# kiranchhatre/amuse

Hardware: AMD Instinct MI355X
Metric: SMPL-X frames/sec (10 s clip, 1000-step DDPM) (higher is better)
Workload: dtype bf16; 1 GPU; 256 x 10 s clips in total (256 on rank 0), DDPM-1000 sampling loop + VAE decode (300 frames) + 6D->axis-angle; random-init weights of the diff_latent_v2 / prior_emotional_fing architecture; clips_total=256, clips_rank0=256, clips_per_tile=2, sampler=ddpm-1000, mfma_operands=bf16, state_and_accumulate=fp32

## Files before the change

### amuse_amd/csrc/amuse_sample8.hpp

```cpp
#pragma once
#include "amuse_dev.hpp"
#include "amuse_kernels.hpp"

namespace amuse {
namespace {

constexpr int kR8 = kRing8;
using Ring = WRing<kR8>;
constexpr int kA8Bytes = 8 * kTiles * 64 * 16;
constexpr int kStat8Off = kA8Bytes;

__device__ __forceinline__ f32x4* a8_slot(char* lds, int row, int col, int lane) {
    return reinterpret_cast<f32x4*>(lds) + (row * kTiles + col) * 64 + lane;
}
__device__ __forceinline__ constexpr int part_row(int w, int t) {
    const int red = 4 + (t >> 1);
    const int k = w - (w > red ? 1 : 0);
    return k + (k >= t ? 1 : 0);
}
__device__ __forceinline__ f32x4* u_slot(char* lds, int t, int lane) { return a8_slot(lds, t == 6 ? 5 : 6, t, lane); }

struct Prof8 {
    unsigned long long* out;
    int idx;
    bool on;
};
template <bool PROF>
__device__ __forceinline__ void stamp8(Prof8& pf) {
    if constexpr (PROF) {
        if (pf.on) pf.out[pf.idx++] = __builtin_readcyclecounter();
    }
}

struct Lane8 {
    int lane, g, r, cl, tok;
    long clip;
    bool valid, is_lat;
};
__device__ __forceinline__ Lane8 lane_info(const SampleKernelArgs& a, int lane) {
    asm volatile("" : "+v"(lane));
    Lane8 L;
    L.lane = lane;
    L.g = lane >> 4;
    L.r = lane & 15;
    const int S = a.S, R = S * a.G;
    L.cl = L.r / S;
    L.tok = L.r - L.cl * S;
    L.clip = (long)blockIdx.x * a.G + L.cl;
    L.valid = (L.r < R) && (L.clip < (long)a.B);
    L.is_lat = L.valid && L.tok == 0;
    return L;
}

__device__ __forceinline__ void store_tap_tile(float* tap, int slot, int t, const f32x4& v, int g, int r) {
    st4(tap + ((size_t)slot * 16 + r) * kD + 16 * t + 4 * g, v);
}

__device__ __forceinline__ bool key_valid8(const Lane8& L0, int j, int S, int R) {
    return L0.valid ? (j < R && (j / S) == L0.cl) : (j == L0.r);
}

__device__ __forceinline__ float2 row_stats32(const f32x4 (&y)[2]) {
    float s = ((y[0][0] + y[0][1]) + (y[0][2] + y[0][3])) + ((y[1][0] + y[1][1]) + (y[1][2] + y[1][3]));
    s = allreduce_g_sum(s);
    const float mw = s * (1.0f / 32.0f);
    float m2 = 0.f;
#pragma unroll
    for (int i = 0; i < 2; ++i)
#pragma unroll
        for (int m = 0; m < 4; ++m) {
            const float d = y[i][m] - mw;
            m2 += d * d;
        }
    m2 = allreduce_g_sum(m2);
    return float2{mw, m2};
}
template <bool FAST>
__device__ __forceinline__ float2 row_stats_merge(const float2* stats, int r) {
    const float2 s0 = stats[r], s1 = stats[16 + r], s2 = stats[32 + r], s3 = stats[48 + r];
    const float mean = ((s0.x + s1.x) + (s2.x + s3.x)) * 0.25f;
    const float d0 = s0.x - mean, d1 = s1.x - mean, d2 = s2.x - mean, d3 = s3.x - mean;
    const float M2 = ((s0.y + s1.y) + (s2.y + s3.y)) + 32.0f * ((d0 * d0 + d1 * d1) + (d2 * d2 + d3 * d3));
    const float var = M2 * (1.0f / kD) + 1e-5f;
    return float2{mean, FAST ? __builtin_amdgcn_rsqf(var) : 1.0f / sqrtf(var)};
}

template <class Args>
__device__ __forceinline__ f32x4 static_row4(const Args& a, const Lane8& L, int f) {
    f32x4 sv = splat4(0.f);
    if (L.valid) {
        if (L.tok == 0) sv = ld4(a.pe0 + f);
        else if (L.tok >= 2) sv = ld4(a.cond_tok + ((size_t)L.clip * (a.S - 2) + (L.tok - 2)) * kD + f);
    }
    return sv;
}
template <class Args>
__device__ __forceinline__ f32x4 init_latent4(const Args& a, const Lane8& L, int t, int f) {
    f32x4 l0 = splat4(0.f);
    if (L.is_lat)
        l0 = a.x_init ? ld4(a.x_init + (size_t)L.clip * kD + f)
                      : counter_normal4(a.seed, a.clip0 + (uint64_t)L.clip, 0u, (uint32_t)(4 * t + L.g), 0u);
    return l0;
}
template <class Args>
__device__ __forceinline__ f32x4 assemble_tile(const Args& a, const Lane8& L, int lane, int g, const f32x4* tokrows, const float* ttl,
                                               const f32x4* latl, int step, int t) {
    const f32x4 sv = tokrows[t * 64 + lane];
    f32x4 tt = ld4(ttl + (step & 1) * kD + 16 * t + 4 * g);
    if (a.time_tok_clip) tt = ld4(a.time_tok_clip + (size_t)(L.valid ? L.clip : 0) * kD + 16 * t + 4 * g);
    return !L.valid ? splat4(0.f) : (L.tok == 0 ? latl[t * 64 + lane] + sv : (L.tok == 1 ? tt : sv));
}

}
}
```

### amuse_amd/csrc/k_sampler8.hip

```cpp
#include "amuse_sample8.hpp"

#ifdef AMUSE_OP_F16
#define OPV f16x8
#define OP_PACK pack_f16
#define OP_MFMA mfma_f16
#define OP_PREC PREC_F16
#define OP_GELU gelu_poly4h
#define OP_KERNEL k_sample8h
#define OP_LAUNCH launch_sample8h
#else
#define OPV bf16x8
#define OP_PACK pack_bf16
#define OP_MFMA mfma_bf16
#define OP_PREC PREC_BF16
#define OP_GELU gelu_poly4
#define OP_KERNEL k_sample8
#define OP_LAUNCH launch_sample8
#endif

namespace amuse {

namespace {

constexpr int kSkip8Off = kStat8Off + 8 * 16 * 8;
// ... 44 lines not shown
            ga[i] = ld4(gamma + 16 * (T0 + i) + 4 * g);
            be[i] = ld4(beta + 16 * (T0 + i) + 4 * g);
        }
    }
    __syncthreads();
    f32x4 y[2];
    {
        f32x4 p[NP][2];
#pragma unroll
        for (int i = 0; i < 2; ++i)
#pragma unroll
            for (int w = 0; w < NP; ++w) {
                if (w != 4 + W) p[w][i] = *a8_slot(lds, part_row(w, T0 + i), T0 + i, lane);
            }
#pragma unroll
        for (int i = 0; i < 2; ++i) {
            f32x4 sum;
            if constexpr (NP == 8) {
                p[4 + W][i] = part[T0 + i];
                sum = ((p[0][i] + p[1][i]) + (p[2][i] + p[3][i])) + ((p[4][i] + p[5][i]) + (p[6][i] + p[7][i]));
            } else {
                sum = ((p[0][i] + p[1][i]) + p[2][i]) + p[3][i];
            }
            f32x4 br = sum + bi[i];
            if constexpr (DRP) br = sdrop_apply4(br, dbits >> (4 * i), dscale);
            y[i] = LN ? xo[i] + br : br;
        }
    }
    if constexpr (LN) {
    const float2 st = row_stats32(y);
    if (g == 0) stats[W * 16 + r] = st;
    __syncthreads();
    const float2 ms = row_stats_merge<FAST>(stats, r);
    const float mean = ms.x, rstd = ms.y;
#pragma unroll
    for (int i = 0; i < 2; ++i)
#pragma unroll
        for (int m = 0; m < 4; ++m) y[i][m] = (y[i][m] - mean) * rstd * ga[i][m] + be[i][m];
    }
    xo[0] = y[0];
    xo[1] = y[1];
    xb[W] = OP_PACK(y[0], y[1]);
    *xb_slot(lds, W, lane) = __builtin_bit_cast(uint4, xb[W]);
    __syncthreads();
#pragma unroll
    for (int c = 0; c < 4; ++c)
        if (c != W) xb[c] = __builtin_bit_cast(OPV, *xb_slot(lds, c, lane));
    asm volatile("; combine_red case %0" ::"n"(W));
}
template <int NP, bool FAST, bool LN = true, bool DRP = false>
__device__ __forceinline__ void combine_reduce(f32x4 (&part)[kTiles], f32x4 (&xo)[2], OPV (&xb)[4],
                                               const float* bias, const float* gamma, const float* beta, char* lds,
                                               int h, int lane, uint32_t dbits = 0, float dscale = 1.f) {
    if (h == 0) combine_red<0, NP, FAST, LN, DRP>(part, xo, xb, bias, gamma, beta, lds, lane, dbits, dscale);
    else if (h == 1) combine_red<1, NP, FAST, LN, DRP>(part, xo, xb, bias, gamma, beta, lds, lane, dbits, dscale);
    else if (h == 2) combine_red<2, NP, FAST, LN, DRP>(part, xo, xb, bias, gamma, beta, lds, lane, dbits, dscale);
    else combine_red<3, NP, FAST, LN, DRP>(part, xo, xb, bias, gamma, beta, lds, lane, dbits, dscale);
}
struct NoHook {
    __device__ void operator()() const {}
};
template <int N0, int N1, int N2, int N3, int IPH0, bool LN = true, class Hook = NoHook>
__device__ __forceinline__ void combine_publish(const f32x4 (&part)[kTiles], OPV (&xb)[4], char* lds, int h,
                                                int lane, Ring& rg, Hook hook = {}) {
#pragma unroll
    for (int t = 0; t < kTiles; ++t)
        *a8_slot(lds, h + (h >= t ? 1 : 0), t, lane) = part[t];
    ring_issue<N0, kR8, IPH0 % kR8>(rg);
    __syncthreads();
    ring_issue<N1, kR8, (IPH0 + N0) % kR8>(rg);
    hook();
    if constexpr (LN) __syncthreads();
    ring_issue<N2, kR8, (IPH0 + N0 + N1) % kR8>(rg);
    __syncthreads();
#pragma unroll
    for (int c = 0; c < 4; ++c) xb[c] = __builtin_bit_cast(OPV, *xb_slot(lds, c, lane));
    ring_issue<N3, kR8, (IPH0 + N0 + N1 + N2) % kR8>(rg);
}

template <int N0, int N1, int N2>
__device__ __forceinline__ void combine_publish_c2(const f32x4 (&part)[kTiles], OPV (&xb)[4], char* lds, int h,
                                                   int lane, Ring& rg, bool skip_u, const uint4* skip_ops) {
    static_assert(N0 >= 8 && N0 + N1 + N2 == 32, "the leading 8 units go out before the first barrier");
#pragma unroll
    for (int t = 0; t < kTiles; ++t)
        *a8_slot(lds, h + (h >= t ? 1 : 0), t, lane) = part[t];
    ring_issue<N0, kR8, 24>(rg);
    __syncthreads();
    ring_issue<N1, kR8, (24 + N0) % kR8>(rg);
    __syncthreads();
    if (skip_u) {
        OPV sk[4];
#pragma unroll
        for (int p = 0; p < 4; ++p) sk[p] = __builtin_bit_cast(OPV, skip_ops[p * 64 + lane]);
        f32x4 u[2] = {splat4(0.f), splat4(0.f)};
        gemm_xb<2, false, 24>(u, sk, rg);
        *u_slot(lds, 2 * h, lane) = u[0];
        *u_slot(lds, 2 * h + 1, lane) = u[1];
    }
    ring_issue<N2, kR8, (24 + N0 + N1) % kR8>(rg);
    __syncthreads();
#pragma unroll
    for (int c = 0; c < 4; ++c) xb[c] = __builtin_bit_cast(OPV, *xb_slot(lds, c, lane));
}

template <bool DROP = false>
__device__ __forceinline__ void attention_head8(const f32x4 (&q)[2], const f32x4 (&k)[2], const f32x4 (&v)[2],
                                                const bool (&kvalid)[4], f32x4 (&o)[2], uint32_t dbits = 0,
                                                float dscale = 1.f) {
    f32x4 st = OP_MFMA(OP_PACK(k[0], k[1]), OP_PACK(q[0], q[1]), splat4(0.f));
    float mx = -INFINITY;
#pragma unroll
    for (int m = 0; m < 4; ++m) mx = kvalid[m] ? fmaxf(mx, st[m]) : mx;
    mx = allreduce_g_max(mx);
    f32x4 p;
    float sum = 0.f;
#pragma unroll
    for (int m = 0; m < 4; ++m) {
        const float e = __builtin_amdgcn_exp2f(1.44269504088896340736f * (st[m] - mx));
        p[m] = kvalid[m] ? e : 0.f;
        sum += p[m];
    }
    sum = allreduce_g_sum(sum);
    const float inv = __builtin_amdgcn_rcpf(sum);
#pragma unroll
    for (int m = 0; m < 4; ++m) p[m] *= inv;
    if constexpr (DROP) p = sdrop_apply4(p, dbits, dscale);
#pragma unroll
    for (int td = 0; td < 2; ++td)
        o[td] = OP_MFMA(OP_PACK(v[td], splat4(0.f)), OP_PACK(p, splat4(0.f)), splat4(0.f));
}

template <bool DROP>
__device__ __forceinline__ void gelu_pair(f32x4 (&hq)[2], uint32_t dbits, float dscale) {
    hq[0] = OP_GELU(hq[0]);
    hq[1] = OP_GELU(hq[1]);
    if constexpr (DROP) {
        hq[0] = sdrop_apply4(hq[0], dbits, dscale);
        hq[1] = sdrop_apply4(hq[1], dbits >> 4, dscale);
    }
}

template <int Q0, int NLATE, bool DROP = false>
__device__ __forceinline__ void ffn_half(f32x4 (&part)[kTiles], const OPV (&xb)[4], Ring& rg, const float* pv,
                                         int h, int g, uint32_t dbits = 0, float dscale = 1.f) {
    constexpr int P = OP_PREC;
    const float* b1 = pv + PV_L1_B + 16 * (kTiles * h + 2 * Q0) + 4 * g;
    f32x4 ha[2] = {ld4(b1), ld4(b1 + 16)}, hb[2] = {ld4(b1 + 32), ld4(b1 + 48)};
    gemm_xb<2, false, 0>(ha, xb, rg);
    ring_issue<NLATE, kR8, 32 - NLATE>(rg);
    __builtin_amdgcn_sched_barrier(0);
    gemm_xb<2, false, 8>(hb, xb, rg);
    gelu_pair<DROP>(ha, dbits, dscale);
#pragma unroll
    for (int i = 0; i < 8; ++i) {
        __builtin_amdgcn_sched_group_barrier(0x008, 1, 0);
        __builtin_amdgcn_sched_group_barrier(0x002, kFfnValuPerMfma, 0);
    }
    __builtin_amdgcn_sched_barrier(0);
    gemm_ring<P, kTiles, 2, false, kR8, 16, false>(part, ha, rg);
    gelu_pair<DROP>(hb, dbits >> 8, dscale);
#pragma unroll
    for (int i = 0; i < 8; ++i) {
        __builtin_amdgcn_sched_group_barrier(0x008, 1, 0);
        __builtin_amdgcn_sched_group_barrier(0x002, kFfnValuPerMfma, 0);
    }
    __builtin_amdgcn_sched_barrier(0);
    gemm_ring<P, kTiles, 2, false, kR8, 24, false>(part, hb, rg);
}

struct SDrop8 {
    uint64_t seed;
    uint32_t step, epoch2, thr;
    float scale;
};
template <bool DROP, class Args>
__device__ __forceinline__ SDrop8 sdrop8_of(const Args& a) {
    SDrop8 d{};
    if constexpr (DROP) {
        d.seed = a.drop_seed; d.epoch2 = 2u + *a.drop_epoch; d.thr = a.drop_thr; d.scale = a.drop_scale;
    }
    return d;
}
__device__ __forceinline__ uint32_t sdrop8_attn_bits(const SampleKernelArgs& a, const SDrop8& d, int blk, int h, int lane) {
    const Lane8 L = lane_info(a, lane);
    const int S = a.S, base = (h * S + L.tok) * S + 4 * L.g - L.cl * S, e4 = base >> 2;
    const uint32_t cu = (uint32_t)(a.clip0 + (uint64_t)L.clip), ls = 4u * blk;
    const uint32_t b = sdrop_bits4(d.seed, cu, d.step, ls, (uint32_t)e4 & 0xffffu, d.epoch2, d.thr) |
                       (sdrop_bits4(d.seed, cu, d.step, ls, (uint32_t)(e4 + 1) & 0xffffu, d.epoch2, d.thr) << 4);
    return b >> (base - 4 * e4);
}
template <int Q0>
__device__ __forceinline__ uint32_t sdrop8_ffn_bits(const SampleKernelArgs& a, const SDrop8& d, int blk, int h, int lane) {
    const Lane8 L = lane_info(a, lane);
    const uint32_t cu = (uint32_t)(a.clip0 + (uint64_t)L.clip), e4 = (uint32_t)(L.tok * 128 + 4 * (kTiles * h + 2 * Q0) + L.g);
    uint32_t b = 0;
#pragma unroll
    for (int k = 0; k < 4; ++k) b |= sdrop_bits4(d.seed, cu, d.step, 4u * blk + 2u, e4 + 4 * k, d.epoch2, d.thr) << (4 * k);
    return b;
}
__device__ __forceinline__ uint32_t sdrop8_row_bits(const SampleKernelArgs& a, const SDrop8& d, uint32_t ls, int h, int lane) {
    const Lane8 L = lane_info(a, lane);
    const uint32_t cu = (uint32_t)(a.clip0 + (uint64_t)L.clip), e4 = (uint32_t)(L.tok * 32 + 8 * h + L.g);
    return sdrop_bits4(d.seed, cu, d.step, ls, e4, d.epoch2, d.thr) | (sdrop_bits4(d.seed, cu, d.step, ls, e4 + 4, d.epoch2, d.thr) << 4);
}

template <bool ROLEA, bool PROF, bool DROP, class Early = NoHook>
__device__ __forceinline__ void encoder_block8(OPV (&xb)[4], f32x4 (&xo)[2], Ring& rg, const float* pv,
                                               const bool (&kvalid)[4], char* lds, int h, int lane, bool next_has_skip,
                                               const uint4* skip_next, Prof8& pf, const SampleKernelArgs& a,
                                               const SDrop8& dr, int blk, Early early = {}) {
    constexpr int P = OP_PREC;
    const int g = lane >> 4, r = lane & 15;
    f32x4 part[kTiles];
    if constexpr (ROLEA) {
        uint32_t abits = 0, fbits = 0;
        if constexpr (DROP) abits = sdrop8_attn_bits(a, dr, blk, h, lane);
        f32x4 b_qk[4];
        float b_v[2];
#pragma unroll
        for (int o = 0; o < 2; ++o) {
            b_qk[o] = ld4(pv + PV_IN_B + 16 * (2 * h + o) + 4 * g);
            b_qk[2 + o] = ld4(pv + PV_IN_B + kD + 16 * (2 * h + o) + 4 * g);
            b_v[o] = pv[PV_IN_B + 2 * kD + 16 * (2 * h + o) + r];
        }
        f32x4 qk[4], v[2];
#pragma unroll
        for (int o = 0; o < 4; ++o) qk[o] = splat4(0.f);
        v[0] = v[1] = splat4(0.f);
        gemm_xb<4, false, 0>(qk, xb, rg);
        gemm_xb<2, true, 16>(v, xb, rg);
        const float scaling = 0.17677669529663687f;
        f32x4 q[2] = {(qk[0] + b_qk[0]) * scaling, (qk[1] + b_qk[1]) * scaling};
        f32x4 k[2] = {qk[2] + b_qk[2], qk[3] + b_qk[3]};
        v[0] += splat4(b_v[0]);
        v[1] += splat4(b_v[1]);
        f32x4 o[2];
        attention_head8<DROP>(q, k, v, kvalid, o, abits, dr.scale);
#pragma unroll
        for (int t = 0; t < kTiles; ++t) part[t] = splat4(0.f);
        gemm_ring<P, kTiles, 2, false, kR8, 24, false>(part, o, rg);
        stamp8<PROF>(pf);
        if constexpr (DROP) {
            auto hook = [&]() { fbits = sdrop8_ffn_bits<0>(a, dr, blk, h, lane); };
            combine_publish<0, kC1N1, kC1N2, 32 - kC1N1 - kC1N2 - kALate, 0, true, decltype(hook)>(part, xb, lds, h, lane, rg, hook);
        } else {
            combine_publish<0, kC1N1, kC1N2, 32 - kC1N1 - kC1N2 - kALate, 0>(part, xb, lds, h, lane, rg);
        }
        stamp8<PROF>(pf);
#pragma unroll
        for (int t = 0; t < kTiles; ++t) part[t] = splat4(0.f);
        ffn_half<0, kALate, DROP>(part, xb, rg, pv, h, g, fbits, dr.scale);
        stamp8<PROF>(pf);
        combine_publish_c2<kC2N0, kC2N1, 32 - kC2N0 - kC2N1>(part, xb, lds, h, lane, rg, next_has_skip, skip_next);
    } else {
        ring_issue<kBEarly, kR8, 0>(rg);
        early();
        uint32_t bbits = 0;
        if constexpr (DROP)
            bbits = sdrop8_row_bits(a, dr, 4u * blk + 1u, h, lane) | (sdrop8_row_bits(a, dr, 4u * blk + 3u, h, lane) << 8) |
                    (sdrop8_ffn_bits<2>(a, dr, blk, h, lane) << 16);
        stamp8<PROF>(pf);
#pragma unroll
        for (int t = 0; t < kTiles; ++t) part[t] = splat4(0.f);
        combine_reduce<4, true, true, DROP>(part, xo, xb, pv + PV_OUT_B, pv + PV_LN1_W, pv + PV_LN1_B, lds, h, lane, bbits, dr.scale);
        stamp8<PROF>(pf);
        ffn_half<2, 32 - kBEarly, DROP>(part, xb, rg, pv, h, g, bbits >> 16, dr.scale);
        stamp8<PROF>(pf);
        if (next_has_skip) ring_issue<8, kR8, 0>(rg);
        combine_reduce<8, true, true, DROP>(part, xo, xb, pv + PV_L2_B, pv + PV_LN2_W, pv + PV_LN2_B, lds, h, lane, bbits >> 8, dr.scale);
    }
    stamp8<PROF>(pf);
}

template <bool ROLEA, bool PROF, bool DROP, class Args>
__device__ __forceinline__ void role_loop8(const Args& a, char* smem, int w8, const Lane8& L0) {
    uint4* skipbf = reinterpret_cast<uint4*>(smem + kSkip8Off);
    const float* pvl = reinterpret_cast<const float*>(smem + kPv8Off);
    const f32x4* tokrows = reinterpret_cast<const f32x4*>(smem + kTokRows8Off);
    f32x4* latl = reinterpret_cast<f32x4*>(smem + kLat8Off);
    float* ttl = reinterpret_cast<float*>(smem + kTT8Off);
    float2* stats = reinterpret_cast<float2*>(smem + kStat8Off);
    const float* pv_skip = pvl + kLayers * kEncPv;
    const float* pv_final = pv_skip + 4 * kD;
    const int lane = L0.lane, g = L0.g, r = L0.r, h = w8 & 3;
    const int S = a.S, R = S * a.G;
    bool kvalid[4];
#pragma unroll
    for (int m = 0; m < 4; ++m) kvalid[m] = key_valid8(L0, 4 * g + m, S, R);
    const bool tap = !ROLEA && a.tap_out != nullptr && blockIdx.x == 0;
    const uint32_t wbase_units = ROLEA ? (uint32_t)w8 * (a.wave_units_a + kR8)
                                       : 4u * (a.wave_units_a + kR8) + (uint32_t)(w8 - 4) * a.wave_units_b;
    const uint4* wbase = a.wstream + (size_t)wbase_units * 64 + lane;
    Ring rg;
    if constexpr (ROLEA) {
#pragma unroll
        for (int i = 0; i < kR8; ++i) rg.s[(24 + i) % kR8] = ldw(wbase + i * 64);
        rg.next = wbase + kR8 * 64;
    } else {
        ring_fill(rg, wbase);
    }
    Prof8 pf{a.prof_out ? a.prof_out + (size_t)w8 * 96 : nullptr, 0, false};
    SDrop8 dr = sdrop8_of<DROP>(a);
#pragma unroll 1
    for (int step = 0; step < a.T; ++step) {
        dr.step = (uint32_t)step;
        OPV xb[4];
        f32x4 xo[2] = {splat4(0.f), splat4(0.f)};
        f32x4 zn[2] = {splat4(0.f), splat4(0.f)};
        {
            const Lane8 L = lane_info(a, lane);
            auto assemble = [&](int t) { return assemble_tile(a, L, lane, g, tokrows, ttl, latl, step, t); };
#pragma unroll
            for (int c = 0; c < 4; ++c) xb[c] = OP_PACK(assemble(2 * c), assemble(2 * c + 1));
            if constexpr (!ROLEA) {
                xo[0] = assemble(2 * h);
                xo[1] = assemble(2 * h + 1);
            }
        }
        if (tap && step == 0) {
            store_tap_tile(a.tap_out, 0, 2 * h, xo[0], g, r);
            store_tap_tile(a.tap_out, 0, 2 * h + 1, xo[1], g, r);
        }
        if (!ROLEA && w8 == 4 && lane < 32 && step + 1 < a.T)
            st4(ttl + ((step + 1) & 1) * kD + 4 * lane, ld4(a.time_tok + (size_t)(step + 1) * kD + 4 * lane));
        if constexpr (PROF) {
            pf.on = a.prof_out != nullptr && blockIdx.x == 0 && lane == 0 && step == a.prof_step;
            pf.idx = 0;
        }
        stamp8<PROF>(pf);
        rg.next = ROLEA ? wbase + kR8 * 64 : wbase;
#pragma unroll 1
        for (int blk = 0; blk < kLayers; ++blk) {
            if (blk >= 5) {
                if constexpr (ROLEA) {
                    ring_issue<8, kR8, 24>(rg);
                } else {
                    const float* bs = pv_skip + (blk - 5) * kD + 32 * h + 4 * g;
                    f32x4 acc[2] = {ld4(bs) + *u_slot(smem, 2 * h, lane), ld4(bs + 16) + *u_slot(smem, 2 * h + 1, lane)};
                    gemm_xb<2, false, 0>(acc, xb, rg);
                    xo[0] = acc[0];
                    xo[1] = acc[1];
                    *reinterpret_cast<uint4*>(a8_slot(smem, 7, h, lane)) = __builtin_bit_cast(uint4, OP_PACK(acc[0], acc[1]));
                }
                __syncthreads();
#pragma unroll
                for (int c = 0; c < 4; ++c) xb[c] = __builtin_bit_cast(OPV, *reinterpret_cast<const uint4*>(a8_slot(smem, 7, c, lane)));
            }
            stamp8<PROF>(pf);
            auto early = [&]() {
                if constexpr (!ROLEA && !DROP) {
                    if (blk == kLayers - 1 && !a.no_update && !a.step_noise) {
                        const Lane8 L = lane_info(a, lane);
                        if (a.coef[(size_t)step * 8 + 5] != 0.f && L.is_lat) {
#pragma unroll
                            for (int i = 0; i < 2; ++i)
                                zn[i] = counter_normal4(a.seed, a.clip0 + (uint64_t)L.clip, (uint32_t)step, (uint32_t)(4 * (2 * h + i) + L.g), 1u);
                        }
                    }
                }
            };
            encoder_block8<ROLEA, PROF, DROP, decltype(early)>(xb, xo, rg, pvl + blk * kEncPv, kvalid, smem, h, lane, blk >= 4 && blk < kLayers - 1,
                                                               skipbf + (7 - blk) * 4 * 64, pf, a, dr, blk, early);
            if (!ROLEA && blk < 4 && w8 == 4) {
#pragma unroll
                for (int p = 0; p < 4; ++p) skipbf[(blk * 4 + p) * 64 + lane] = __builtin_bit_cast(uint4, xb[p]);
            }
            if (tap && step == 0) {
                store_tap_tile(a.tap_out, 1 + blk, 2 * h, xo[0], g, r);
                store_tap_tile(a.tap_out, 1 + blk, 2 * h + 1, xo[1], g, r);
            }
        }
        if constexpr (!ROLEA) {
            const float* cf = a.coef + (size_t)step * 8;
            const float sb = cf[0], sa = cf[1], c0 = cf[2], cx = cf[3], ce = cf[4], sg = cf[5], clipv = cf[6];
            const float2 st = row_stats32(xo);
            if (g == 0) stats[h * 16 + r] = st;
            __syncthreads();
            const Lane8 L = lane_info(a, lane);
            f32x4 ga[2], be[2], l[2];
#pragma unroll
            for (int i = 0; i < 2; ++i) {
                ga[i] = ld4(pv_final + 16 * (2 * h + i) + 4 * L.g);
                be[i] = ld4(pv_final + kD + 16 * (2 * h + i) + 4 * L.g);
                l[i] = latl[(2 * h + i) * 64 + L.lane];
            }
            const float2 ms = row_stats_merge<true>(stats, L.r);
            const float inv_sa = 1.0f / sa;
            f32x4 e[2];
#pragma unroll
            for (int i = 0; i < 2; ++i)
#pragma unroll
                for (int m = 0; m < 4; ++m) e[i][m] = (xo[i][m] - ms.x) * ms.y * ga[i][m] + be[i][m];
#pragma unroll
            for (int i = 0; i < 2; ++i) {
                const int t = 2 * h + i, f = 16 * t + 4 * L.g;
                if (tap && step == 0) store_tap_tile(a.tap_out, 10, t, e[i], L.g, L.r);
                if (a.eps_out && L.is_lat && step == a.T - 1) st4(a.eps_out + (size_t)L.clip * kD + f, e[i]);
            }
            if (!a.no_update) {
                f32x4 z[2] = {zn[0], zn[1]};
                if (sg != 0.f && L.is_lat && (DROP || a.step_noise)) {
#pragma unroll
                    for (int i = 0; i < 2; ++i) {
                        const int t = 2 * h + i, f = 16 * t + 4 * L.g;
                        z[i] = a.step_noise ? ld4(a.step_noise + ((size_t)step * a.B + L.clip) * kD + f)
                                            : counter_normal4(a.seed, a.clip0 + (uint64_t)L.clip, (uint32_t)step, (uint32_t)(4 * t + L.g), 1u);
                    }
                }
#pragma unroll
                for (int i = 0; i < 2; ++i)
#pragma unroll
                    for (int m = 0; m < 4; ++m) l[i][m] = sched_update<true>(l[i][m], e[i][m], z[i][m], sb, sa, c0, cx, ce, sg, clipv, inv_sa);
#pragma unroll
                for (int i = 0; i < 2; ++i) {
                    const int t = 2 * h + i, f = 16 * t + 4 * L.g;
                    latl[t * 64 + L.lane] = l[i];
                    if (a.traj_out && L.is_lat) st4(a.traj_out + ((size_t)step * a.B + L.clip) * kD + f, l[i]);
                }
            }
        } else {
            __syncthreads();
        }
        stamp8<PROF>(pf);
        __syncthreads();
    }
}

template <bool PROF, bool DROP, class Args>
__global__ __launch_bounds__(512) void OP_KERNEL(Args a) {
    extern __shared__ __attribute__((aligned(16))) char smem[];
    float* pvl = reinterpret_cast<float*>(smem + kPv8Off);
    f32x4* tokrows = reinterpret_cast<f32x4*>(smem + kTokRows8Off);
    f32x4* latl = reinterpret_cast<f32x4*>(smem + kLat8Off);
    float* ttl = reinterpret_cast<float*>(smem + kTT8Off);
    for (int i = threadIdx.x; i < kLayers * kEncPv / 4; i += 512) {
        const int blk = (4 * i) / kEncPv, off = 4 * i - blk * kEncPv;
        st4(pvl + 4 * i, ld4(a.pvec + blk * PV_BLOCK + off));
    }
    for (int i = threadIdx.x; i < (4 * kD + 2 * kD) / 4; i += 512) st4(pvl + kLayers * kEncPv + 4 * i, ld4(a.pvec + PV_SKIP_B + 4 * i));
    const int w8 = __builtin_amdgcn_readfirstlane(threadIdx.x >> 6);
    const Lane8 L = lane_info(a, threadIdx.x & 63);
    if (w8 == 0) {
#pragma unroll
        for (int t = 0; t < kTiles; ++t) {
            const int f = 16 * t + 4 * L.g;
            const f32x4 sv = static_row4(a, L, f), l0 = init_latent4(a, L, t, f);
            tokrows[t * 64 + L.lane] = sv;
            latl[t * 64 + L.lane] = l0;
        }
    }
    if (w8 == 4 && L.lane < 32 && !a.time_tok_clip) st4(ttl + 4 * L.lane, ld4(a.time_tok + 4 * L.lane));
    __syncthreads();
    if (w8 < 4) role_loop8<true, PROF, DROP>(a, smem, w8, L);
    else role_loop8<false, PROF, DROP>(a, smem, w8, L);
    if (L.is_lat && w8 == 0 && a.latents_out) {
#pragma unroll
        for (int t = 0; t < kTiles; ++t) st4(a.latents_out + (size_t)L.clip * kD + 16 * t + 4 * L.g, latl[t * 64 + L.lane]);
    }
}

}

hipError_t OP_LAUNCH(const SampleArgs& a_in, hipStream_t stream) {
    SampleArgs a = a_in;
    if (a.drop_thr > 0 && !(a.drop_epoch = train_epoch_ptr())) return hipErrorOutOfMemory;
    const int tiles = (a.B + a.G - 1) / a.G;
    static DeviceOnce once;
    int dev_;
    if (!once.done(&dev_)) {
        for (const void* k : {reinterpret_cast<const void*>(&OP_KERNEL<false, false, SampleKernelArgs>), reinterpret_cast<const void*>(&OP_KERNEL<true, false, SampleKernelArgs>),
                              reinterpret_cast<const void*>(&OP_KERNEL<false, true, SampleArgs>), reinterpret_cast<const void*>(&OP_KERNEL<true, true, SampleArgs>)}) {
            hipError_t e = hipFuncSetAttribute(k, hipFuncAttributeMaxDynamicSharedMemorySize, kSample8LdsBytes);
            if (e != hipSuccess) return e;
        }
        once.set(dev_);
    }
    const SampleKernelArgs ka = a;
    if (a.drop_thr > 0) {
        if (a.prof_out) hipLaunchKernelGGL((OP_KERNEL<true, true, SampleArgs>), dim3(tiles), dim3(512), kSample8LdsBytes, stream, a);
        else hipLaunchKernelGGL((OP_KERNEL<false, true, SampleArgs>), dim3(tiles), dim3(512), kSample8LdsBytes, stream, a);
    } else if (a.prof_out) hipLaunchKernelGGL((OP_KERNEL<true, false, SampleKernelArgs>), dim3(tiles), dim3(512), kSample8LdsBytes, stream, ka);
    else hipLaunchKernelGGL((OP_KERNEL<false, false, SampleKernelArgs>), dim3(tiles), dim3(512), kSample8LdsBytes, stream, ka);
    return hipGetLastError();
}

}
```

### amuse_amd/csrc/k_sampler8x.hip

```cpp
#include "amuse_sample8.hpp"

namespace amuse {

namespace {

constexpr int kPvSlotFloats = 7 * 256;
static_assert(kPvSlotFloats >= kEncPv && kPvSlotFloats <= PV_BLOCK, "a slot is filled by whole pieces read from the block's own region");
constexpr int kPv8Off = kStat8Off + 8 * 16 * 8;
constexpr int kPvTail8Off = kPv8Off + 2 * kPvSlotFloats * 4;
constexpr int kSkip8Off = kPvTail8Off + (4 * kD + 2 * kD) * 4;
constexpr int kTokRows8Off = kSkip8Off + 4 * 8 * 64 * 16;
constexpr int kLat8Off = kTokRows8Off + kTiles * 64 * 16;
constexpr int kTT8Off = kLat8Off + kTiles * 64 * 16;
static_assert(kTT8Off + 2 * kD * 4 == kSample8xLdsBytes, "LDS layout");

constexpr int kXC1N1 = 12, kXC1N2 = 12, kXC2N1 = 8;
constexpr int kXBEarly = 32;
constexpr int kXBPrio = 3;

__device__ __forceinline__ uint4* xs_hi_slot(char* lds, int c, int lane) { return reinterpret_cast<uint4*>(a8_slot(lds, c, c, lane)); }
__device__ __forceinline__ uint4* xs_lo_slot(char* lds, int c, int lane) { return reinterpret_cast<uint4*>(a8_slot(lds, 4 + c, 4 + c, lane)); }
__device__ __forceinline__ void publish_xs(char* lds, int c, int lane, const F16Pair& p) {
    *xs_hi_slot(lds, c, lane) = __builtin_bit_cast(uint4, p.hi);
    *xs_lo_slot(lds, c, lane) = __builtin_bit_cast(uint4, p.lo);
// ... 15 lines not shown
            const int s0 = (PH + 2 * (c * NO + o)) % kR8, s1 = (PH + 2 * (c * NO + o) + 1) % kR8;
            wh[o] = __builtin_bit_cast(f16x8, rg.s[s0]);
            wl[o] = __builtin_bit_cast(f16x8, rg.s[s1]);
            if constexpr (REARM) {
                rg.s[s0] = ldw(rg.next);
                rg.s[s1] = ldw_pos(rg.next + 64, 1);
                rg.next += 128;
            }
        }
#pragma unroll
        for (int o = 0; o < NO; ++o) acc[o] = SWAP ? mfma_f16(xs[c].hi, wl[o], acc[o]) : mfma_f16(wl[o], xs[c].hi, acc[o]);
#pragma unroll
        for (int o = 0; o < NO; ++o) acc[o] = SWAP ? mfma_f16(xs[c].lo, wh[o], acc[o]) : mfma_f16(wh[o], xs[c].lo, acc[o]);
#pragma unroll
        for (int o = 0; o < NO; ++o) acc[o] = SWAP ? mfma_f16(xs[c].hi, wh[o], acc[o]) : mfma_f16(wh[o], xs[c].hi, acc[o]);
    }
}

template <int W, int NP>
__device__ __forceinline__ void combine_red(f32x4 (&part)[kTiles], f32x4 (&xo)[2], F16Pair (&xs)[4], const float* bias,
                                            const float* gamma, const float* beta, char* lds, int lane) {
    float2* stats = reinterpret_cast<float2*>(lds + kStat8Off);
    const int g = lane >> 4, r = lane & 15;
    constexpr int T0 = 2 * W;
    if constexpr (NP == 8) {
#pragma unroll
        for (int t = 0; t < kTiles; ++t)
            if (t != T0 && t != T0 + 1) *a8_slot(lds, part_row(4 + W, t), t, lane) = part[t];
    }
    f32x4 bi[2], ga[2], be[2];
#pragma unroll
    for (int i = 0; i < 2; ++i) {
        bi[i] = ld4(bias + 16 * (T0 + i) + 4 * g);
        ga[i] = ld4(gamma + 16 * (T0 + i) + 4 * g);
        be[i] = ld4(beta + 16 * (T0 + i) + 4 * g);
    }
    __syncthreads();
    f32x4 y[2];
    {
        f32x4 p[NP][2];
#pragma unroll
        for (int i = 0; i < 2; ++i)
#pragma unroll
            for (int w = 0; w < NP; ++w)
                if (w != 4 + W) p[w][i] = *a8_slot(lds, part_row(w, T0 + i), T0 + i, lane);
#pragma unroll
        for (int i = 0; i < 2; ++i) {
            f32x4 sum;
            if constexpr (NP == 8) {
                p[4 + W][i] = part[T0 + i];
                sum = ((p[0][i] + p[1][i]) + (p[2][i] + p[3][i])) + ((p[4][i] + p[5][i]) + (p[6][i] + p[7][i]));
            } else {
                sum = ((p[0][i] + p[1][i]) + p[2][i]) + p[3][i];
            }
            y[i] = xo[i] + (sum + bi[i]);
        }
    }
    const float2 st = row_stats32(y);
    if (g == 0) stats[W * 16 + r] = st;
    __syncthreads();
    const float2 ms = row_stats_merge<false>(stats, r);
    const float mean = ms.x, rstd = ms.y;
#pragma unroll
    for (int i = 0; i < 2; ++i)
#pragma unroll
        for (int m = 0; m < 4; ++m) y[i][m] = (y[i][m] - mean) * rstd * ga[i][m] + be[i][m];
    xo[0] = y[0];
    xo[1] = y[1];
    xs[W] = split_f16(y[0], y[1]);
    publish_xs(lds, W, lane, xs[W]);
    __syncthreads();
#pragma unroll
    for (int c = 0; c < 4; ++c)
        if (c != W) xs[c] = gather_xs(lds, c, lane);
    asm volatile("; combine_red case %0" ::"n"(W));
}
template <int NP>
__device__ __forceinline__ void combine_reduce(f32x4 (&part)[kTiles], f32x4 (&xo)[2], F16Pair (&xs)[4], const float* bias,
                                               const float* gamma, const float* beta, char* lds, int h, int lane) {
    if (h == 0) combine_red<0, NP>(part, xo, xs, bias, gamma, beta, lds, lane);
    else if (h == 1) combine_red<1, NP>(part, xo, xs, bias, gamma, beta, lds, lane);
    else if (h == 2) combine_red<2, NP>(part, xo, xs, bias, gamma, beta, lds, lane);
    else combine_red<3, NP>(part, xo, xs, bias, gamma, beta, lds, lane);
}

__device__ __forceinline__ uint4* sk_hi_slot(char* lds, int c, int lane) { return reinterpret_cast<uint4*>(a8_slot(lds, 7, c, lane)); }
__device__ __forceinline__ uint4* sk_lo_slot(char* lds, int c, int lane) { return reinterpret_cast<uint4*>(a8_slot(lds, 5, c, lane)); }

template <int N1, int N2>
__device__ __forceinline__ void combine_publish_c1(const f32x4 (&part)[kTiles], F16Pair (&xs)[4], char* lds, int h, int lane,
                                                   Ring& rg, bool push, uint4* skip_dst, const float* pv_next_src, unsigned pv_next_dst) {
#pragma unroll
    for (int t = 0; t < kTiles; ++t) *a8_slot(lds, h + (h >= t ? 1 : 0), t, lane) = part[t];
    if (push) {
        if (h == 0) { skip_dst[0 * 64] = __builtin_bit_cast(uint4, xs[0].hi); skip_dst[1 * 64] = __builtin_bit_cast(uint4, xs[0].lo); }
        else if (h == 1) { skip_dst[2 * 64] = __builtin_bit_cast(uint4, xs[1].hi); skip_dst[3 * 64] = __builtin_bit_cast(uint4, xs[1].lo); }
        else if (h == 2) { skip_dst[4 * 64] = __builtin_bit_cast(uint4, xs[2].hi); skip_dst[5 * 64] = __builtin_bit_cast(uint4, xs[2].lo); }
        else { skip_dst[6 * 64] = __builtin_bit_cast(uint4, xs[3].hi); skip_dst[7 * 64] = __builtin_bit_cast(uint4, xs[3].lo); }
    }
    __syncthreads();
    {
        const uint4* src = reinterpret_cast<const uint4*>(pv_next_src) + (2 * h) * 64 + lane;
        const unsigned dst = __builtin_amdgcn_readfirstlane(pv_next_dst + (2 * h) * 1024);
        glds16(src, dst);
        if (h < 3) glds16(src + 64, dst + 1024);
    }
    ring_issue<N1, kR8, 0>(rg);
    __syncthreads();
    ring_issue<N2, kR8, N1>(rg);
    __syncthreads();
#pragma unroll
    for (int c = 0; c < 4; ++c) xs[c] = gather_xs(lds, c, lane);
    ring_issue<32 - N1 - N2, kR8, N1 + N2>(rg);
}

template <int N1>
__device__ __forceinline__ void combine_publish_c2(const f32x4 (&part)[kTiles], F16Pair (&xs)[4], char* lds, int h, int lane,
                                                   Ring& rg, bool skip_u, const uint4* skip_src) {
#pragma unroll
    for (int t = 0; t < kTiles; ++t) *a8_slot(lds, h + (h >= t ? 1 : 0), t, lane) = part[t];
    F16Pair sk[4];
    if (skip_u) {
#pragma unroll
        for (int c = 0; c < 4; ++c) {
            sk[c].hi = __builtin_bit_cast(f16x8, skip_src[(2 * c) * 64]);
            sk[c].lo = __builtin_bit_cast(f16x8, skip_src[(2 * c + 1) * 64]);
        }
    }
    ring_issue<16, kR8, 0>(rg);
    __syncthreads();
    ring_issue<N1, kR8, 16>(rg);
    __syncthreads();
    if (skip_u) {
        f32x4 u[2] = {splat4(0.f), splat4(0.f)};
        gemm_xs<2, 4, false, 0, false>(u, sk, rg);
        *u_slot(lds, 2 * h, lane) = u[0];
        *u_slot(lds, 2 * h + 1, lane) = u[1];
    }
    ring_issue<16 - N1, kR8, 16 + N1>(rg);
    __syncthreads();
#pragma unroll
    for (int c = 0; c < 4; ++c) xs[c] = gather_xs(lds, c, lane);
}

__device__ __forceinline__ void attention_head8x(const f32x4 (&q)[2], const f32x4 (&k)[2], const f32x4 (&v)[2],
                                                 const bool (&kvalid)[4], f32x4 (&o)[2]) {
    const F16Pair ks = split_f16(k[0], k[1]), qs = split_f16(q[0], q[1]);
    f32x4 st = mfma_f16(ks.lo, qs.hi, splat4(0.f));
    st = mfma_f16(ks.hi, qs.lo, st);
    st = mfma_f16(ks.hi, qs.hi, st);
    float mx = -INFINITY;
#pragma unroll
    for (int m = 0; m < 4; ++m) mx = kvalid[m] ? fmaxf(mx, st[m]) : mx;
    mx = allreduce_g_max(mx);
    f32x4 p;
    float sum = 0.f;
#pragma unroll
    for (int m = 0; m < 4; ++m) {
        const float e = expf(st[m] - mx);
        p[m] = kvalid[m] ? e : 0.f;
        sum += p[m];
    }
    sum = allreduce_g_sum(sum);
#pragma unroll
    for (int m = 0; m < 4; ++m) p[m] = p[m] / sum;
    const F16Pair ps = split_f16(p, splat4(0.f));
#pragma unroll
    for (int td = 0; td < 2; ++td) {
        const F16Pair vs = split_f16(v[td], splat4(0.f));
        o[td] = mfma_f16(vs.lo, ps.hi, splat4(0.f));
        o[td] = mfma_f16(vs.hi, ps.lo, o[td]);
        o[td] = mfma_f16(vs.hi, ps.hi, o[td]);
    }
}

__device__ __forceinline__ void gelu_pair(f32x4 (&hq)[2]) {
#pragma unroll
    for (int i = 0; i < 2; ++i)
#pragma unroll
        for (int m = 0; m < 4; ++m) {
            hq[i][m] = gelu_erf(hq[i][m]);
        }
}

template <int Q0, int EARLY, bool DEFER, bool PROF>
__device__ __forceinline__ void ffn_half(f32x4 (&part)[kTiles], const F16Pair (&xs)[4], Ring& rg, const float* pv, int h, int g, Prof8& pf) {
    const float* b1 = pv + PV_L1_B + 16 * (kTiles * h + 2 * Q0) + 4 * g;
    f32x4 ha[2] = {ld4(b1), ld4(b1 + 16)}, hb[2] = {ld4(b1 + 32), ld4(b1 + 48)};
    if constexpr (EARLY < 32) ring_issue<32 - EARLY, kR8, EARLY>(rg);
    gemm_xs<2, 4, false, 0, !DEFER>(ha, xs, rg);
    stamp8<PROF>(pf);
    gemm_xs<2, 4, false, 16, !DEFER>(hb, xs, rg);
    stamp8<PROF>(pf);
    gelu_pair(ha);
    stamp8<PROF>(pf);
    if constexpr (DEFER) {
        gelu_pair(hb);
        ring_issue<32, kR8, 0>(rg);
        stamp8<PROF>(pf);
        const F16Pair hsa = split_f16(ha[0], ha[1]), hsb = split_f16(hb[0], hb[1]);
        gemm_xs<kTiles, 1, false, 0, false>(part, &hsa, rg);
        stamp8<PROF>(pf);
        gemm_xs<kTiles, 1, false, 16, false>(part, &hsb, rg);
    } else {
        {
            const F16Pair hs = split_f16(ha[0], ha[1]);
            gemm_xs<kTiles, 1, false, 0, false>(part, &hs, rg);
        }
        stamp8<PROF>(pf);
        gelu_pair(hb);
        stamp8<PROF>(pf);
        const F16Pair hs = split_f16(hb[0], hb[1]);
        gemm_xs<kTiles, 1, false, 16, false>(part, &hs, rg);
    }
}

template <bool ROLEA, bool PROF>
__device__ __forceinline__ void encoder_block8x(F16Pair (&xs)[4], f32x4 (&xo)[2], Ring& rg, const float* pv,
                                                const bool (&kvalid)[4], char* lds, int h, int lane, bool push, uint4* skip_dst,
                                                bool next_has_skip, const uint4* skip_src, const float* pv_next_src, unsigned pv_next_dst,
                                                Prof8& pf) {
    const int g = lane >> 4, r = lane & 15;
    f32x4 part[kTiles];
    if constexpr (ROLEA) {
        f32x4 b_qk[4];
        float b_v[2];
#pragma unroll
        for (int o = 0; o < 2; ++o) {
            b_qk[o] = ld4(pv + PV_IN_B + 16 * (2 * h + o) + 4 * g);
            b_qk[2 + o] = ld4(pv + PV_IN_B + kD + 16 * (2 * h + o) + 4 * g);
            b_v[o] = pv[PV_IN_B + 2 * kD + 16 * (2 * h + o) + r];
        }
        f32x4 qk[4], v[2];
#pragma unroll
        for (int o = 0; o < 4; ++o) qk[o] = splat4(0.f);
        v[0] = v[1] = splat4(0.f);
        gemm_xs<4, 2, false, 16, true>(qk, xs, rg);
        gemm_xs<2, 4, true, 0, true>(v, xs, rg);
        gemm_xs<4, 2, false, 16, false>(qk, xs + 2, rg);
        const float scaling = 0.17677669529663687f;
        f32x4 q[2] = {(qk[0] + b_qk[0]) * scaling, (qk[1] + b_qk[1]) * scaling};
        f32x4 k[2] = {qk[2] + b_qk[2], qk[3] + b_qk[3]};
        v[0] += splat4(b_v[0]);
        v[1] += splat4(b_v[1]);
        f32x4 o[2];
        attention_head8x(q, k, v, kvalid, o);
#pragma unroll
        for (int t = 0; t < kTiles; ++t) part[t] = splat4(0.f);
        {
            const F16Pair os = split_f16(o[0], o[1]);
            gemm_xs<kTiles, 1, false, 0, false>(part, &os, rg);
        }
        stamp8<PROF>(pf);
        combine_publish_c1<kXC1N1, kXC1N2>(part, xs, lds, h, lane, rg, push, skip_dst, pv_next_src, pv_next_dst);
        stamp8<PROF>(pf);
#pragma unroll
        for (int t = 0; t < kTiles; ++t) part[t] = splat4(0.f);
        ffn_half<0, 32, true, PROF>(part, xs, rg, pv, h, g, pf);
        stamp8<PROF>(pf);
        combine_publish_c2<kXC2N1>(part, xs, lds, h, lane, rg, next_has_skip, skip_src);
    } else {
        ring_issue<kXBEarly, kR8, 0>(rg);
        stamp8<PROF>(pf);
#pragma unroll
        for (int t = 0; t < kTiles; ++t) part[t] = splat4(0.f);
        combine_reduce<4>(part, xo, xs, pv + PV_OUT_B, pv + PV_LN1_W, pv + PV_LN1_B, lds, h, lane);
        stamp8<PROF>(pf);
        __builtin_amdgcn_s_setprio(kXBPrio);
        ffn_half<2, kXBEarly, false, PROF>(part, xs, rg, pv, h, g, pf);
        __builtin_amdgcn_s_setprio(0);
        stamp8<PROF>(pf);
        if (next_has_skip) ring_issue<16, kR8, 0>(rg);
        combine_reduce<8>(part, xo, xs, pv + PV_L2_B, pv + PV_LN2_W, pv + PV_LN2_B, lds, h, lane);
    }
    stamp8<PROF>(pf);
}

template <bool ROLEA, bool PROF>
__device__ __forceinline__ void role_loop8x(const SampleKernelArgs& a, char* smem, int w8, const Lane8& L0) {
    const float* pvl = reinterpret_cast<const float*>(smem + kPv8Off);
    const f32x4* tokrows = reinterpret_cast<const f32x4*>(smem + kTokRows8Off);
    f32x4* latl = reinterpret_cast<f32x4*>(smem + kLat8Off);
    float* ttl = reinterpret_cast<float*>(smem + kTT8Off);
    float2* stats = reinterpret_cast<float2*>(smem + kStat8Off);
    const float* pv_skip = reinterpret_cast<const float*>(smem + kPvTail8Off);
    const float* pv_final = pv_skip + 4 * kD;
    const int lane = L0.lane, g = L0.g, r = L0.r, h = w8 & 3;
    const int S = a.S, R = S * a.G;
    bool kvalid[4];
#pragma unroll
    for (int m = 0; m < 4; ++m) kvalid[m] = key_valid8(L0, 4 * g + m, S, R);
    const bool tap = !ROLEA && a.tap_out != nullptr && blockIdx.x == 0;
    const uint32_t wbase_units = ROLEA ? (uint32_t)w8 * (a.wave_units_a + kR8)
                                       : 4u * (a.wave_units_a + kR8) + (uint32_t)(w8 - 4) * a.wave_units_b;
    const uint4* wbase = a.wstream + (size_t)wbase_units * 64 + lane;
    uint4* skipl = reinterpret_cast<uint4*>(smem + kSkip8Off) + lane;
    const unsigned pv_lds0 = lds_addr(smem + kPv8Off);
    int gblk = 0;
    Ring rg;
    ring_fill(rg, wbase);
    Prof8 pf{a.prof_out ? a.prof_out + (size_t)w8 * 96 : nullptr, 0, false};
#pragma unroll 1
    for (int step = 0; step < a.T; ++step) {
        F16Pair xs[4];
        f32x4 xo[2] = {splat4(0.f), splat4(0.f)};
        {
            const Lane8 L = lane_info(a, lane);
            auto assemble = [&](int t) { return assemble_tile(a, L, lane, g, tokrows, ttl, latl, step, t); };
#pragma unroll
            for (int c = 0; c < 4; ++c) xs[c] = split_f16(assemble(2 * c), assemble(2 * c + 1));
            if constexpr (!ROLEA) {
                xo[0] = assemble(2 * h);
                xo[1] = assemble(2 * h + 1);
            }
        }
        if (tap && step == 0) {
            store_tap_tile(a.tap_out, 0, 2 * h, xo[0], g, r);
            store_tap_tile(a.tap_out, 0, 2 * h + 1, xo[1], g, r);
        }
        if (!ROLEA && w8 == 4 && lane < 32 && step + 1 < a.T)
            st4(ttl + ((step + 1) & 1) * kD + 4 * lane, ld4(a.time_tok + (size_t)(step + 1) * kD + 4 * lane));
        if constexpr (PROF) {
            pf.on = a.prof_out != nullptr && blockIdx.x == 0 && lane == 0 && step == a.prof_step;
            pf.idx = 0;
        }
        stamp8<PROF>(pf);
        rg.next = ROLEA ? wbase + kR8 * 64 : wbase;
#pragma unroll 1
        for (int blk = 0; blk < kLayers; ++blk) {
            if (blk >= 5) {
                if constexpr (ROLEA) {
                    ring_issue<16, kR8, 0>(rg);
                } else {
                    const float* bs = pv_skip + (blk - 5) * kD + 32 * h + 4 * g;
                    f32x4 acc[2] = {ld4(bs) + *u_slot(smem, 2 * h, lane), ld4(bs + 16) + *u_slot(smem, 2 * h + 1, lane)};
                    gemm_xs<2, 4, false, 0, false>(acc, xs, rg);
                    xo[0] = acc[0];
                    xo[1] = acc[1];
                    const F16Pair pr = split_f16(acc[0], acc[1]);
                    *sk_hi_slot(smem, h, lane) = __builtin_bit_cast(uint4, pr.hi);
                    *sk_lo_slot(smem, h, lane) = __builtin_bit_cast(uint4, pr.lo);
                }
                __syncthreads();
#pragma unroll
                for (int c = 0; c < 4; ++c) {
                    xs[c].hi = __builtin_bit_cast(f16x8, *sk_hi_slot(smem, c, lane));
                    xs[c].lo = __builtin_bit_cast(f16x8, *sk_lo_slot(smem, c, lane));
                }
            }
            stamp8<PROF>(pf);
            const int nblk = blk + 1 == kLayers ? 0 : blk + 1;
            encoder_block8x<ROLEA, PROF>(xs, xo, rg, pvl + (gblk & 1) * kPvSlotFloats, kvalid, smem, h, lane, blk >= 1 && blk <= 4,
                                         skipl + (blk - 1) * 8 * 64, blk >= 4 && blk < kLayers - 1, skipl + (7 - blk) * 8 * 64,
                                         a.pvec + nblk * PV_BLOCK, pv_lds0 + ((gblk + 1) & 1) * (kPvSlotFloats * 4), pf);
            ++gblk;
            if (tap && step == 0) {
                store_tap_tile(a.tap_out, 1 + blk, 2 * h, xo[0], g, r);
                store_tap_tile(a.tap_out, 1 + blk, 2 * h + 1, xo[1], g, r);
            }
        }
        if constexpr (!ROLEA) {
            const float2 st = row_stats32(xo);
            if (g == 0) stats[h * 16 + r] = st;
        }
        __syncthreads();
        if constexpr (!ROLEA) {
            const Lane8 L = lane_info(a, lane);
            const float2 ms = row_stats_merge<false>(stats, L.r);
            const float* cf = a.coef + (size_t)step * 8;
            const float sb = cf[0], sa = cf[1], c0 = cf[2], cx = cf[3], ce = cf[4], sg = cf[5], clipv = cf[6];
            const float inv_sa = 1.0f / sa;
#pragma unroll
            for (int i = 0; i < 2; ++i) {
                const int t = 2 * h + i, f = 16 * t + 4 * L.g;
                const f32x4 ga = ld4(pv_final + f), be = ld4(pv_final + kD + f);
                f32x4 e;
#pragma unroll
                for (int m = 0; m < 4; ++m) e[m] = (xo[i][m] - ms.x) * ms.y * ga[m] + be[m];
                if (tap && step == 0) store_tap_tile(a.tap_out, 10, t, e, L.g, L.r);
                if (a.eps_out && L.is_lat && step == a.T - 1) st4(a.eps_out + (size_t)L.clip * kD + f, e);
                if (!a.no_update) {
                    f32x4 z = splat4(0.f);
                    if (sg != 0.f && L.is_lat)
                        z = a.step_noise ? ld4(a.step_noise + ((size_t)step * a.B + L.clip) * kD + f)
                                         : counter_normal4(a.seed, a.clip0 + (uint64_t)L.clip, (uint32_t)step, (uint32_t)(4 * t + L.g), 1u);
                    f32x4 l = latl[t * 64 + L.lane];
#pragma unroll
                    for (int m = 0; m < 4; ++m) l[m] = sched_update<false>(l[m], e[m], z[m], sb, sa, c0, cx, ce, sg, clipv, inv_sa);
                    latl[t * 64 + L.lane] = l;
                    if (a.traj_out && L.is_lat) st4(a.traj_out + ((size_t)step * a.B + L.clip) * kD + f, l);
                }
            }
        }
        stamp8<PROF>(pf);
        __syncthreads();
    }
}

template <bool PROF>
__global__ __launch_bounds__(512) void k_sample8x(SampleKernelArgs a) {
    extern __shared__ __attribute__((aligned(16))) char smem[];
    float* pvl = reinterpret_cast<float*>(smem + kPv8Off);
    f32x4* tokrows = reinterpret_cast<f32x4*>(smem + kTokRows8Off);
    f32x4* latl = reinterpret_cast<f32x4*>(smem + kLat8Off);
    float* ttl = reinterpret_cast<float*>(smem + kTT8Off);
    for (int i = threadIdx.x; i < kEncPv / 4; i += 512) st4(pvl + 4 * i, ld4(a.pvec + 4 * i));
    for (int i = threadIdx.x; i < (4 * kD + 2 * kD) / 4; i += 512)
        st4(reinterpret_cast<float*>(smem + kPvTail8Off) + 4 * i, ld4(a.pvec + PV_SKIP_B + 4 * i));
    const int w8 = __builtin_amdgcn_readfirstlane(threadIdx.x >> 6);
    const Lane8 L = lane_info(a, threadIdx.x & 63);
    if (w8 == 0) {
#pragma unroll
        for (int t = 0; t < kTiles; ++t) {
            const int f = 16 * t + 4 * L.g;
            const f32x4 sv = static_row4(a, L, f), l0 = init_latent4(a, L, t, f);
            tokrows[t * 64 + L.lane] = sv;
            latl[t * 64 + L.lane] = l0;
        }
    }
    if (w8 == 4 && L.lane < 32 && !a.time_tok_clip) st4(ttl + 4 * L.lane, ld4(a.time_tok + 4 * L.lane));
    __syncthreads();
    if (w8 < 4) role_loop8x<true, PROF>(a, smem, w8, L);
    else role_loop8x<false, PROF>(a, smem, w8, L);
    if (L.is_lat && w8 == 0 && a.latents_out) {
#pragma unroll
        for (int t = 0; t < kTiles; ++t) st4(a.latents_out + (size_t)L.clip * kD + 16 * t + 4 * L.g, latl[t * 64 + L.lane]);
    }
}

}

hipError_t launch_sample8x(const SampleArgs& a, hipStream_t stream) {
    const int tiles = (a.B + a.G - 1) / a.G;
    static DeviceOnce once;
    int dev_;
    if (!once.done(&dev_)) {
        for (const void* k : {reinterpret_cast<const void*>(&k_sample8x<false>), reinterpret_cast<const void*>(&k_sample8x<true>)}) {
            hipError_t e = hipFuncSetAttribute(k, hipFuncAttributeMaxDynamicSharedMemorySize, kSample8xLdsBytes);
            if (e != hipSuccess) return e;
        }
        once.set(dev_);
    }
    if (a.prof_out) hipLaunchKernelGGL(k_sample8x<true>, dim3(tiles), dim3(512), kSample8xLdsBytes, stream, static_cast<const SampleKernelArgs&>(a));
    else hipLaunchKernelGGL(k_sample8x<false>, dim3(tiles), dim3(512), kSample8xLdsBytes, stream, static_cast<const SampleKernelArgs&>(a));
    return hipGetLastError();
}

}
```

Before: 2.296 million frames/s.

## Assemble next-step input tiles at end of step and share via LDS

In the bf16 sampler, each B-role wave now assembles only its own two input tiles at the end of the previous step and publishes them packed to an LDS slot. All waves then read the four packed tiles from LDS instead of each wave rebuilding all eight tiles from token rows, time tokens and latents. The time_tok_clip path is folded into the static token rows, and the fp16 variant's assembly is restructured into branch-light batched loads. This removes redundant per-wave assembly work from the step's critical path, at the cost of extra LDS traffic and a dependence on existing barriers for correctness. Profiling stamp placement also changes.

```diff
diff --git a/amuse_amd/csrc/amuse_sample8.hpp b/amuse_amd/csrc/amuse_sample8.hpp
--- a/amuse_amd/csrc/amuse_sample8.hpp
+++ b/amuse_amd/csrc/amuse_sample8.hpp
@@ -91,6 +91,7 @@
     if (L.valid) {
         if (L.tok == 0) sv = ld4(a.pe0 + f);
         else if (L.tok >= 2) sv = ld4(a.cond_tok + ((size_t)L.clip * (a.S - 2) + (L.tok - 2)) * kD + f);
+        else if (a.time_tok_clip) sv = ld4(a.time_tok_clip + (size_t)L.clip * kD + f);
     }
     return sv;
 }
@@ -102,13 +103,35 @@
                       : counter_normal4(a.seed, a.clip0 + (uint64_t)L.clip, 0u, (uint32_t)(4 * t + L.g), 0u);
     return l0;
 }
+struct TokSrc {
+    const f32x4* x;
+    int stride;
+    bool is_lat;
+};
 template <class Args>
-__device__ __forceinline__ f32x4 assemble_tile(const Args& a, const Lane8& L, int lane, int g, const f32x4* tokrows, const float* ttl,
-                                               const f32x4* latl, int step, int t) {
-    const f32x4 sv = tokrows[t * 64 + lane];
-    f32x4 tt = ld4(ttl + (step & 1) * kD + 16 * t + 4 * g);
-    if (a.time_tok_clip) tt = ld4(a.time_tok_clip + (size_t)(L.valid ? L.clip : 0) * kD + 16 * t + 4 * g);
-    return !L.valid ? splat4(0.f) : (L.tok == 0 ? latl[t * 64 + lane] + sv : (L.tok == 1 ? tt : sv));
+__device__ __forceinline__ TokSrc tok_src(const Args& a, const Lane8& L, int lane, int g, const f32x4* tokrows, const float* ttl, int step) {
+    const bool from_tt = L.valid && L.tok == 1 && !a.time_tok_clip;
+    return TokSrc{from_tt ? reinterpret_cast<const f32x4*>(ttl + (step & 1) * kD) + g : tokrows + lane, from_tt ? 4 : 64, L.is_lat};
+}
+__device__ __forceinline__ f32x4 assemble_pick(const TokSrc& s, const f32x4& x, const f32x4& la) {
+    const f32x4 sum = la + x;
+    return s.is_lat ? sum : x;
+}
+template <int N>
+__device__ __forceinline__ void assemble_load(f32x4 (&x)[N], f32x4 (&la)[N], const TokSrc& s, const f32x4* latl, int lane, int T0) {
+#pragma unroll
+    for (int i = 0; i < N; ++i) {
+        x[i] = s.x[(T0 + i) * s.stride];
+        la[i] = latl[(T0 + i) * 64 + lane];
+    }
+}
+template <class Args>
+__device__ __forceinline__ void assemble_own(f32x4 (&xo)[2], const f32x4 (&la)[2], const Args& a, const Lane8& L, const f32x4* tokrows, const float* ttl,
+                                             int step, int h) {
+    const TokSrc s = tok_src(a, L, L.lane, L.g, tokrows, ttl, step);
+    const f32x4 x0 = s.x[(2 * h) * s.stride], x1 = s.x[(2 * h + 1) * s.stride];
+    xo[0] = assemble_pick(s, x0, la[0]);
+    xo[1] = assemble_pick(s, x1, la[1]);
 }
 
 }
diff --git a/amuse_amd/csrc/k_sampler8.hip b/amuse_amd/csrc/k_sampler8.hip
--- a/amuse_amd/csrc/k_sampler8.hip
+++ b/amuse_amd/csrc/k_sampler8.hip
@@ -370,31 +370,31 @@
     }
     Prof8 pf{a.prof_out ? a.prof_out + (size_t)w8 * 96 : nullptr, 0, false};
     SDrop8 dr = sdrop8_of<DROP>(a);
+    f32x4 xo[2] = {splat4(0.f), splat4(0.f)};
+    if constexpr (!ROLEA) {
+        const Lane8 L = lane_info(a, lane);
+        const f32x4 l[2] = {latl[(2 * h) * 64 + L.lane], latl[(2 * h + 1) * 64 + L.lane]};
+        assemble_own(xo, l, a, L, tokrows, ttl, 0, h);
+        *xb_slot(smem, h, L.lane) = __builtin_bit_cast(uint4, OP_PACK(xo[0], xo[1]));
+    }
+    __syncthreads();
 #pragma unroll 1
     for (int step = 0; step < a.T; ++step) {
+        if constexpr (PROF) {
+            stamp8<PROF>(pf);
+            pf.on = a.prof_out != nullptr && blockIdx.x == 0 && lane == 0 && step == a.prof_step;
+            stamp8<PROF>(pf);
+        }
         dr.step = (uint32_t)step;
         OPV xb[4];
-        f32x4 xo[2] = {splat4(0.f), splat4(0.f)};
         f32x4 zn[2] = {splat4(0.f), splat4(0.f)};
-        {
-            const Lane8 L = lane_info(a, lane);
-            auto assemble = [&](int t) { return assemble_tile(a, L, lane, g, tokrows, ttl, latl, step, t); };
-#pragma unroll
-            for (int c = 0; c < 4; ++c) xb[c] = OP_PACK(assemble(2 * c), assemble(2 * c + 1));
-            if constexpr (!ROLEA) {
-                xo[0] = assemble(2 * h);
-                xo[1] = assemble(2 * h + 1);
-            }
-        }
+#pragma unroll
+        for (int c = 0; c < 4; ++c) xb[c] = __builtin_bit_cast(OPV, *xb_slot(smem, c, lane));
+        if (!ROLEA && w8 == 4 && lane < 32 && step + 1 < a.T)
+            st4(ttl + ((step + 1) & 1) * kD + 4 * lane, ld4(a.time_tok + (size_t)(step + 1) * kD + 4 * lane));
         if (tap && step == 0) {
             store_tap_tile(a.tap_out, 0, 2 * h, xo[0], g, r);
             store_tap_tile(a.tap_out, 0, 2 * h + 1, xo[1], g, r);
-        }
-        if (!ROLEA && w8 == 4 && lane < 32 && step + 1 < a.T)
-            st4(ttl + ((step + 1) & 1) * kD + 4 * lane, ld4(a.time_tok + (size_t)(step + 1) * kD + 4 * lane));
-        if constexpr (PROF) {
-            pf.on = a.prof_out != nullptr && blockIdx.x == 0 && lane == 0 && step == a.prof_step;
-            pf.idx = 0;
         }
         stamp8<PROF>(pf);
         rg.next = ROLEA ? wbase + kR8 * 64 : wbase;
@@ -487,6 +487,10 @@
                     if (a.traj_out && L.is_lat) st4(a.traj_out + ((size_t)step * a.B + L.clip) * kD + f, l[i]);
                 }
             }
+            if (step + 1 < a.T) {
+                assemble_own(xo, l, a, L, tokrows, ttl, step + 1, h);
+                *xb_slot(smem, h, L.lane) = __builtin_bit_cast(uint4, OP_PACK(xo[0], xo[1]));
+            }
         } else {
             __syncthreads();
         }
diff --git a/amuse_amd/csrc/k_sampler8x.hip b/amuse_amd/csrc/k_sampler8x.hip
--- a/amuse_amd/csrc/k_sampler8x.hip
+++ b/amuse_amd/csrc/k_sampler8x.hip
@@ -341,27 +341,31 @@
     Prof8 pf{a.prof_out ? a.prof_out + (size_t)w8 * 96 : nullptr, 0, false};
 #pragma unroll 1
     for (int step = 0; step < a.T; ++step) {
+        if constexpr (PROF) {
+            stamp8<PROF>(pf);
+            pf.on = a.prof_out != nullptr && blockIdx.x == 0 && lane == 0 && step == a.prof_step;
+            stamp8<PROF>(pf);
+        }
         F16Pair xs[4];
         f32x4 xo[2] = {splat4(0.f), splat4(0.f)};
         {
             const Lane8 L = lane_info(a, lane);
-            auto assemble = [&](int t) { return assemble_tile(a, L, lane, g, tokrows, ttl, latl, step, t); };
-#pragma unroll
-            for (int c = 0; c < 4; ++c) xs[c] = split_f16(assemble(2 * c), assemble(2 * c + 1));
+            const TokSrc ts = tok_src(a, L, lane, g, tokrows, ttl, step);
+            f32x4 x[kTiles], la[kTiles], xr[2], lr[2];
+            assemble_load<kTiles>(x, la, ts, latl, lane, 0);
+            if constexpr (!ROLEA) assemble_load<2>(xr, lr, ts, latl, lane, 2 * h);
+#pragma unroll
+            for (int c = 0; c < 4; ++c) xs[c] = split_f16(assemble_pick(ts, x[2 * c], la[2 * c]), assemble_pick(ts, x[2 * c + 1], la[2 * c + 1]));
             if constexpr (!ROLEA) {
-                xo[0] = assemble(2 * h);
-                xo[1] = assemble(2 * h + 1);
-            }
-        }
+                xo[0] = assemble_pick(ts, xr[0], lr[0]);
+                xo[1] = assemble_pick(ts, xr[1], lr[1]);
+            }
+        }
+        if (!ROLEA && w8 == 4 && lane < 32 && step + 1 < a.T)
+            st4(ttl + ((step + 1) & 1) * kD + 4 * lane, ld4(a.time_tok + (size_t)(step + 1) * kD + 4 * lane));
         if (tap && step == 0) {
             store_tap_tile(a.tap_out, 0, 2 * h, xo[0], g, r);
             store_tap_tile(a.tap_out, 0, 2 * h + 1, xo[1], g, r);
-        }
-        if (!ROLEA && w8 == 4 && lane < 32 && step + 1 < a.T)
-            st4(ttl + ((step + 1) & 1) * kD + 4 * lane, ld4(a.time_tok + (size_t)(step + 1) * kD + 4 * lane));
-        if constexpr (PROF) {
-            pf.on = a.prof_out != nullptr && blockIdx.x == 0 && lane == 0 && step == a.prof_step;
-            pf.idx = 0;
         }
         stamp8<PROF>(pf);
         rg.next = ROLEA ? wbase + kR8 * 64 : wbase;
```

Measured after the change: 2.369 million frames/s, median of 6. +3.1%, better.
